# gvtulder/elasticdeform

Measured on AMD Instinct MI355X. Metric: Mvoxels/s fwd+grad, 256^3 fp32 order=3, higher is better.
Workload: dtype f32; 1 GPU; cfg2: 3D 256x256x256 float32, 5x5x5 grid sigma 5, order 3, mode mirror, prefilter on, deform_grid + deform_grid_gradient per step, one volume per GPU; parallelism=1 volume per GPU, no collective

## Files before the change

### elasticdeform_amd/csrc/deform_hot.hip

```cpp
#include <hip/hip_runtime.h>

#include <type_traits>

#include "ed_device.h"
#include "ed_params.h"
#include "ed_tile.h"

#ifndef ED_K2_U1
#define ED_K2_U1 1
#endif
#ifndef ED_K2_U2
#define ED_K2_U2 1
#endif
#define ED_PRAGMA(x) _Pragma(#x)
#define ED_UNROLL(n) ED_PRAGMA(unroll n)

namespace ed {
namespace tile {

namespace {

constexpr int kGradBoxBytes = 24 * 1024;

__device__ __forceinline__ void box_reduce_to_lds(int* red, int lane, int (&lo)[3], int (&hi)[3])
{
    box_reduce<6>(lo, hi);
    if (lane == 63) {
        const unsigned addr = (unsigned)(size_t)(__attribute__((address_space(3))) void*)red;
        asm volatile("ds_min_i32 %0, %1\n\t"
                     "ds_min_i32 %0, %2 offset:4\n\t"
                     "ds_min_i32 %0, %3 offset:8\n\t"
                     "ds_max_i32 %0, %4 offset:12\n\t"
                     "ds_max_i32 %0, %5 offset:16\n\t"
                     "ds_max_i32 %0, %6 offset:20"
                     :
                     : "v"(addr), "v"(lo[0]), "v"(lo[1]), "v"(lo[2]), "v"(hi[0]), "v"(hi[1]), "v"(hi[2])
                     : "memory");
    }
}
__device__ __forceinline__ float load_dy(const float* dy, long long off, int io16)
{
    return io16 ? widen16(reinterpret_cast<const unsigned short*>(dy)[off], io16) : dy[off];
}

__device__ __forceinline__ void hot_prologue(const HotGeom& hg, const Strip& sp, char* smem, int tid,
                                             bool copy_q = true, int nthreads = kBlock)
{
    int* sred = reinterpret_cast<int*>(smem + kOffRed);
    {
        const int* src = reinterpret_cast<const int*>(hg.xt + sp.tx0 * kT);
        int* dst = reinterpret_cast<int*>(smem + kOffTabX);
        const int avail = (hg.out_len[2] - sp.tx0 * kT) * 12;
        for (int e = tid; e < kStrip * kT * 12; e += nthreads)
            dst[e] = e < avail ? src[e] : 0;
    }
    if (copy_q && tid < 256) {
        const int row16 = 2 * hg.ncpx;
        const int r = tid >> 2;
        const int oz = min(sp.tz * kT + (r >> 3), hg.out_len[0] - 1);
        const int oy = min(sp.ty * kT + (r & 7), hg.out_len[1] - 1);
        const long long qrow_id = hg.q_strips > 1
                                      ? ((long long)oz * hg.out_len[1] + oy) * hg.q_strips + sp.tx0 / hg.strip_tiles
                                      : (long long)oz * hg.out_len[1] + oy;
        const double2* src = reinterpret_cast<const double2*>(
            hg.q + sp.sample * hg.q_bstride + qrow_id * (4 * hg.ncpx));
        double2* dst = reinterpret_cast<double2*>(smem + kOffQ) + r * row16;
        for (int k = tid & 3; k < row16; k += 4)
            dst[k] = src[k];
    }
    if (tid < 24) {
        const int k = tid & 7;
        sred[tid] = k < 3 ? 0x7fffffff : (int)0x80000000;
    }
    if (tid >= 128 && tid < 128 + 12)
        fill_hot_params(reinterpret_cast<HotParams*>(smem + kOffHot), hg, tid - 128);
    __syncthreads();
}

template <int ORDER, bool AFFINE>
__device__ __forceinline__ bool hot_coords(const HotGeom& hg, const HotParams* hp, const char* qrow,
                                           const double (&tw)[4], const int (&tib)[4], const int (&b)[3],
                                           const double (&P)[3], int* start, float* frac)
{
    double d[3];
    qrow_disp(qrow, tib, tw, d);
    return tile_coords<ORDER, AFFINE, float>(hg.in_len, &hg.mode, hp->period, hp->inv_period, d, b, P, start, frac);
}

template <int ORDER, bool AFFINE, int GRAD_WAVES, int TX, int NGRP = 1, bool IO16 = false>
__global__ __launch_bounds__(kBlock * NGRP, GRAD_WAVES) void hot_grad_kernel(const HotGeom hg)
{
    const int io16 = IO16 ? hg.io16 : 0;
    constexpr int NT = ORDER + 1;
    constexpr int NV = TX / 4, ZSTEP = 8 / NV;
    extern __shared__ __attribute__((aligned(16))) char smem0[];
    const int grp = NGRP == 2 ? (int)(threadIdx.x >> 8) : 0;
    const int tid = threadIdx.x & (kBlock - 1);
    char* smem = smem0 + grp * hg.lds_grp;
    int phase = 0;
    Strip sp;
    const int bidx = NGRP == 2 ? (int)(((blockIdx.x >> 3) * 2 + grp) * 8 + (blockIdx.x & 7)) : (int)blockIdx.x;
    if (!strip_of_block(hg, sp, bidx))
        return;
    for (int e = tid * 4; e < hg.box_cap; e += kBlock * 4)
        *reinterpret_cast<int4*>(smem + hg.off_box + e * 4) = make_int4(0, 0, 0, 0);
    hot_prologue(hg, sp, smem, tid);
    if (ED_DBG(hg.dbg, 8192))
        return;
    if (NGRP == 2 && grp == 1)
        __syncthreads();

    const AxTab* tabx = reinterpret_cast<const AxTab*>(smem + kOffTabX);
    int* sred = reinterpret_cast<int*>(smem + kOffRed);
    const HotParams* hp = reinterpret_cast<const HotParams*>(smem + kOffHot);
    int* box = reinterpret_cast<int*>(smem + hg.off_box);

    const int lane = tid & 63;
    const int wave = tid >> 6;
    const int zq = tid / (TX * 8);
    const bool rows16 = TX == 16 && ED_DBG(hg.dbg, 1 << 21);
    const int xx = (TX == 16 && !rows16) ? 2 * (tid & 7) + ((tid >> 4) & 1) : (tid & (TX - 1));
    const int yy = (TX == 16 && !rows16) ? 4 * ((tid >> 6) & 1) + ((tid >> 5) & 1) + 2 * ((tid >> 3) & 1) : ((tid / TX) & 7);
    const int ntile = (sp.ntile * kT + TX - 1) / TX;
    float* dx = hg.vol_w + sp.sample * hg.vol_bstride;
    const float* __restrict__ dy = hg.img_r + sp.sample * hg.img_bstride;

    const int oy = sp.ty * kT + yy;
    const char* qrow0 = smem + kOffQ + (zq * kT + yy) * (32 * hg.ncpx);
    const int qstep = ZSTEP * kT * 32 * hg.ncpx;
    const int oz0 = sp.tz * kT + zq;
    const bool vy = oy < hg.out_len[1];

    auto load_raw = [&](long long off) -> float {
        if constexpr (IO16)
            return __uint_as_float((unsigned)reinterpret_cast<const unsigned short*>(dy)[off]);
        else
            return dy[off];
    };
    float gnext[NV];
    {
        const int ox = sp.tx0 * kT + xx;
#pragma unroll
        for (int i = 0; i < NV; ++i)
            gnext[i] = (vy && ox < hg.out_len[2] && oz0 + ZSTEP * i < hg.out_len[0])
                           ? load_raw((oz0 + ZSTEP * i) * hg.img_sz + oy * hg.img_sy + ox) : 0.f;
    }
    int half = -1, half_next = -1;
    for (int ti = 0; ti < ntile; half = half_next, half_next = half == 0 ? 1 : -1, ti += half < 0 ? 1 : 0) {
        int* red = sred + (ti % 3) * 8;
        const int ox = sp.tx0 * kT + ti * TX + xx;
        const bool vx = ox < hg.out_len[2];
        const int ooff0 = oz0 * hg.img_sz + oy * hg.img_sy + ox;
        const int ostep = ZSTEP * hg.img_sz;

        float gpre[NV];
        if (half >= 0) {
#pragma unroll
            for (int i = 0; i < NV; ++i)
                gpre[i] = (vy && vx && oz0 + ZSTEP * i < hg.out_len[0]) ? load_raw(ooff0 + i * ostep) : 0.f;
        } else {
#pragma unroll
            for (int i = 0; i < NV; ++i)
                gpre[i] = gnext[i];
        }
        if (half < 0 && ti + 1 < ntile) {
            const bool nvx = ox + TX < hg.out_len[2];
#pragma unroll
            for (int i = 0; i < NV; ++i)
                gnext[i] = (vy && nvx && oz0 + ZSTEP * i < hg.out_len[0]) ? load_raw(ooff0 + TX + i * ostep) : 0.f;
        }
        const bool given = hg.use_boxes != 0;
        int gb0[3] = {0, 0, 0}, gbhi[3] = {-1, -1, -1};
        if (given) {
            const int t0 = sp.sample * hg.ntiles + (sp.tz * hg.tiles[1] + sp.ty) * hg.tiles[2] + sp.tx0 +
                           ti * (TX / kT);
            const int* bx = hg.boxes + (size_t)t0 * 8;
#pragma unroll
            for (int h = 0; h < 3; ++h) {
                gb0[h] = uni(bx[h]);
                gbhi[h] = uni(bx[3 + h]);
            }
            if (half < 0) {
#pragma unroll
                for (int k = 1; k < TX / kT; ++k) {
                    if (sp.tx0 + ti * (TX / kT) + k < hg.tiles[2]) {
#pragma unroll
                        for (int h = 0; h < 3; ++h) {
                            gb0[h] = min(gb0[h], uni(bx[k * 8 + h]));
                            gbhi[h] = max(gbhi[h], uni(bx[k * 8 + 3 + h]));
                        }
                    }
                }
            } else if (half == 1) {
#pragma unroll
                for (int h = 0; h < 3; ++h) {
                    gb0[h] = uni(bx[8 + h]);
                    gbhi[h] = uni(bx[8 + 3 + h]);
                }
            }
        }

        double tw[4];
        int tib[4];
        {
            const AxTab& t = tabx[ti * TX + xx];
#pragma unroll
            for (int l = 0; l < 4; ++l) {
                tw[l] = t.w[l];
                tib[l] = t.idx[l] * 8;
            }
        }
        double Pxy[3] = {0.0, 0.0, 0.0};
        if (AFFINE) {
#pragma unroll
            for (int h = 0; h < 3; ++h)
                Pxy[h] = fma(hp->affine[h * 4 + 2], (double)ox,
                             fma(hp->affine[h * 4 + 1], (double)oy, hp->affine[h * 4 + 3] + hp->offd[h]));
        }
        auto voxel = [&](int i, int* start, float* frac) -> bool {
            const int oz = oz0 + ZSTEP * i;
            const int b[3] = {oz + hg.off[0], oy + hg.off[1], ox + hg.off[2]};
            double P[3] = {0.0, 0.0, 0.0};
            if (AFFINE) {
#pragma unroll
                for (int h = 0; h < 3; ++h)
                    P[h] = fma(hp->affine[h * 4 + 0], (double)oz, Pxy[h]);
            }
            const bool cst = hot_coords<ORDER, AFFINE>(hg, hp, qrow0 + i * qstep, tw, tib, b, P, start, frac);
            return vy && vx && oz < hg.out_len[0] && !cst && (half < 0 || (xx >> 3) == half);
        };
        int lo[3] = {0x7fffffff, 0x7fffffff, 0x7fffffff};
        int hi[3] = {(int)0x80000000, (int)0x80000000, (int)0x80000000};
        if (!given) {
ED_UNROLL(ED_K2_U1)
            for (int i = 0; i < NV; ++i) {
                int start[3];
                float frac[3];
                if (voxel(i, start, frac)) {
#pragma unroll
                    for (int h = 0; h < 3; ++h) {
                        lo[h] = min(lo[h], start[h]);
                        hi[h] = max(hi[h], start[h] + ORDER);
                    }
                }
            }
        }
        float gval[NV];
        {
            float gm = 0.f;
#pragma unroll
            for (int i = 0; i < NV; ++i) {
                gval[i] = IO16 ? widen16(__float_as_uint(gpre[i]), io16) : gpre[i];
                gm += (__float_as_int(gval[i]) & 0x7f800000) == 0x7f800000 ? 0.f : fabsf(gval[i]);
            }
            gm = wave_sum(gm);
            if (lane == 0)
                reinterpret_cast<float*>(smem + kOffSum)[(phase & 1) * 4 + wave] = gm;
        }
        if (!given)
            box_reduce_to_lds(red, lane, lo, hi);
        lds_barrier();
        int b0[3], bhi[3];
        if (given) {
#pragma unroll
            for (int h = 0; h < 3; ++h) {
                b0[h] = gb0[h];
                bhi[h] = gbhi[h];
            }
        } else {
#pragma unroll
            for (int h = 0; h < 3; ++h) {
                b0[h] = uni(red[h]);
                bhi[h] = uni(red[3 + h]);
            }
        }
        bool any = bhi[0] >= b0[0] && bhi[1] >= b0[1] && bhi[2] >= b0[2];
        if (given && !any) {
            b0[0] = b0[1] = b0[2] = 0;
            bhi[0] = bhi[1] = bhi[2] = -1;
            any = true;
        }
        const int ext[3] = {bhi[0] - b0[0] + 1, bhi[1] - b0[1] + 1, bhi[2] - b0[2] + 1};
        if (tid < 6 && !given)
            sred[((ti + 2) % 3) * 8 + tid] = tid < 3 ? 0x7fffffff : (int)0x80000000;
        if (!any)
            continue;
        int pitch = ext[2] <= 8 ? 8 : (ext[2] <= 24 ? 24 : (ext[2] <= 40 ? 40 : (ext[2] <= 56 ? 56 : 0)));
        if (ED_DBG(hg.dbg, 1024))
            pitch = ext[2] <= 16 ? 16 : (ext[2] <= 48 ? 48 : 0);
        if (ED_DBG(hg.dbg, 1 << 22))
            pitch = ext[2] <= 32 ? 32 : 0;
        if (given && ((unsigned)ext[0] > 4096u || (unsigned)ext[1] > 4096u))
            pitch = 0;
        const int by = ext[1];
        const int nrows = ext[0] * by;
        const int nbox = nrows * pitch;
        if (hg.hint && tid == 0 && half < 0 && (pitch == 0 || nbox > hg.small_cap))
            atomicAdd(hg.hint, (hg.large_cap > 0 && (pitch == 0 || nbox > hg.large_cap)) ? kHintHuge * (TX / kT) : TX / kT);
        bool direct_tile = false;
        if (pitch == 0 || nbox > hg.box_cap) {
            if (TX == 16 && given && half < 0 && sp.tx0 + ti * 2 + 1 < hg.tiles[2]) {
                half_next = 0;
                continue;
            }
            if (hg.self_serve) {
                direct_tile = true;
            } else {
                const int t8 = sp.tx0 + ti * (TX / kT) + (half >= 0 ? half : tid);
                if (tid < (half >= 0 ? 1 : TX / kT) && t8 < hg.tiles[2]) {
                    const int slot = atomicAdd(&hg.spill[0], 1);
                    hg.spill[1 + slot] = sp.sample * hg.ntiles + (sp.tz * hg.tiles[1] + sp.ty) * hg.tiles[2] + t8;
                }
                continue;
            }
        }
        const bool interior = b0[0] >= 0 && b0[0] + ext[0] <= hg.in_len[0] && b0[1] >= 0 &&
                              b0[1] + ext[1] <= hg.in_len[1] && b0[2] >= 0 && b0[2] + ext[2] <= hg.in_len[2];

        for (long long ss = 0; ss < hg.nsteps; ++ss, ++phase) {
            long long vol_off = 0, img_off = 0;
            if (hg.nstep)
                hot_step_offsets(hp, ss, vol_off, img_off);
            float* dst = dx + vol_off;
            float* gsum = reinterpret_cast<float*>(smem + kOffSum) + (phase & 1) * 4;
            if (ss > 0) {
                float gm = 0.f;
#pragma unroll
                for (int i = 0; i < NV; ++i) {
                    const bool inb = vy && vx && oz0 + ZSTEP * i < hg.out_len[0];
                    gval[i] = inb ? load_dy(dy, img_off + ooff0 + i * ostep, io16) : 0.f;
                    gm += (__float_as_int(gval[i]) & 0x7f800000) == 0x7f800000 ? 0.f : fabsf(gval[i]);
                }
                gm = wave_sum(gm);
                if (lane == 0)
                    gsum[wave] = gm;
                lds_barrier();
            }
            const float gtot = unif((gsum[0] + gsum[1]) + (gsum[2] + gsum[3]));
            constexpr float kC = (float)((2147483648.0 - 1024.0) /
                                         ((ORDER == 1 ? 1.0 : ORDER == 2 ? 0.4219 : ORDER == 3 ? 0.2963
                                           : ORDER == 4 ? 0.2150 : 0.1664) * 1.001));
            const float scale = gtot > 0.f ? fminf(kC * __frcp_rn(gtot), 3.0e38f) : 0.f;
            const float inv_scale = gtot > 0.f ? __frcp_rn(scale) : 0.f;

ED_UNROLL(ED_K2_U2)
            for (int i = 0; i < NV; ++i) {
                float gv = gval[0];
#pragma unroll
                for (int k = 1; k < NV; ++k)
                    gv = i == k ? gval[k] : gv;
                if (gv == 0.f || ED_DBG(hg.dbg, 128))
                    continue;
                int st[3];
                float fr[3];
                if (!voxel(i, st, fr))
                    continue;
                float w0[NT], w1[NT], w2[NT];
                weights_from_frac<float, ORDER>(fr[0], w0);
                weights_from_frac<float, ORDER>(fr[1], w1);
                weights_from_frac<float, ORDER>(fr[2], w2);
                const int rz = st[0] - b0[0], ry = st[1] - b0[1], rx = st[2] - b0[2];
                const bool outside = direct_tile || (given && (rz < 0 || rz + ORDER >= ext[0] || ry < 0 || ry + ORDER >= ext[1] ||
                                                               rx < 0 || rx + ORDER >= ext[2]));
                if ((__float_as_int(gv) & 0x7f800000) == 0x7f800000 || outside) {
#pragma unroll 1
                    for (int t = 0; t < NT * NT * NT; ++t) {
                        const int l0 = t / (NT * NT), l1 = (t / NT) % NT, l2 = t % NT;
                        const int zs = mirror_i32(st[0] + l0, hg.in_len[0]);
                        const int ys = mirror_i32(st[1] + l1, hg.in_len[1]);
                        const int xs = mirror_i32(st[2] + l2, hg.in_len[2]);
                        float wp = w0[0], wq = w1[0], wr = w2[0];
#pragma unroll
                        for (int l = 1; l < NT; ++l) {
                            wp = l0 == l ? w0[l] : wp;
                            wq = l1 == l ? w1[l] : wq;
                            wr = l2 == l ? w2[l] : wr;
                        }
                        unsafeAtomicAdd(dst + (zs * hg.vol_sz + ys * hg.vol_sy + xs), gv * wp * wq * wr);
                    }
                    continue;
                }
                int* bp = box + (rz * by + ry) * pitch + rx;
                const float gs = gv * scale;
#pragma unroll
                for (int l0 = 0; l0 < NT; ++l0) {
                    const float g0 = gs * w0[l0];
#pragma unroll
                    for (int l1 = 0; l1 < NT; ++l1) {
                        const float g1 = g0 * w1[l1];
                        int* rp = bp + (l0 * by + l1) * pitch;
                        typedef float f2_t __attribute__((ext_vector_type(2)));
                        float pr[NT + 1];
#pragma unroll
                        for (int l2 = 0; l2 + 1 < NT + 1; l2 += 2) {
                            const f2_t wv = {w2[l2], l2 + 1 < NT ? w2[l2 + 1] : 0.f};
                            const f2_t gg = {g1, g1};
                            const f2_t pv = wv * gg;
                            pr[l2] = pv.x;
                            pr[l2 + 1] = pv.y;
                        }
#pragma unroll
                        for (int l2 = 0; l2 < NT; ++l2)
                            atomicAdd(reinterpret_cast<unsigned*>(rp + l2), (unsigned)round_half_up_i32(pr[l2]));
                    }
                }
            }
            lds_barrier();
            {
                constexpr int FL = TX == 8 ? 16 : 32;
                constexpr int FR = kBlock / FL;
                constexpr int FU = 4;
                const int sub = tid & (FL - 1);
                const int rslot = tid / FL;
                const float inv_by = 1.f / (float)by;
                const int nr = (ED_DBG(hg.dbg, 64) || direct_tile) ? 0 : nrows;
                const int dz8 = (int)(((float)FR + 0.5f) * inv_by), dy8 = FR - dz8 * by;
                const int step8 = dz8 * hg.vol_sz + dy8 * hg.vol_sy, wrapfix = hg.vol_sz - by * hg.vol_sy;
                for (int xo = 0; xo < ext[2]; xo += FL) {
                    const int xi = xo + sub;
                    const bool xin = xi < ext[2];
                    const int xs = interior ? xi : mirror_i32(b0[2] + xi, hg.in_len[2]);
                    int zr = (int)(((float)rslot + 0.5f) * inv_by), yr = rslot - zr * by;
                    int rowoff = (b0[0] + zr) * hg.vol_sz + (b0[1] + yr) * hg.vol_sy + b0[2];
                    for (int r0 = rslot; r0 < nr; r0 += FU * FR) {
                        int acc[FU];
#pragma unroll
                        for (int k = 0; k < FU; ++k) {
                            const int r = r0 + k * FR;
                            acc[k] = (xin && r < nr) ? __hip_atomic_exchange(&box[r * pitch + xi], 0, __ATOMIC_RELAXED,
                                                                             __HIP_MEMORY_SCOPE_WORKGROUP)
                                                     : 0;
                        }
#pragma unroll
                        for (int k = 0; k < FU; ++k) {
                            if (ED_DBG(hg.dbg, 4096) ? acc[k] == 0x7ffffff1 : acc[k] != 0) {
                                int off = rowoff;
                                if (!interior)
                                    off = mirror_i32(b0[0] + zr, hg.in_len[0]) * hg.vol_sz +
                                          mirror_i32(b0[1] + yr, hg.in_len[1]) * hg.vol_sy;
                                unsafeAtomicAdd(dst + (off + xs), (float)acc[k] * inv_scale);
                            }
                            yr += dy8;
                            zr += dz8;
                            rowoff += step8;
                            if (yr >= by) {
                                yr -= by;
                                zr += 1;
                                rowoff += wrapfix;
                            }
                        }
                    }
                }
            }
        }
    }
}

template <int ORDER>
hipError_t launch_grad_order(const HotGeom& hg, unsigned nblk, size_t lds, hipStream_t stream)
{
#ifdef EDHIP_EXPERIMENTS
    const int duo = ed_env("EDHIP_GRAD_DUO") ? atoi(ed_env("EDHIP_GRAD_DUO")) : 0;
    if (duo && !hg.has_affine && ORDER == 3) {
        if constexpr (ORDER == 3) {
            auto kern = hot_grad_kernel<ORDER, false, 4, 16, 2>;
            static bool once = false;
            if (!once) {
                (void)hipFuncSetAttribute(reinterpret_cast<const void*>(kern),
                                          hipFuncAttributeMaxDynamicSharedMemorySize, 160 * 1024);
                once = true;
            }
            const unsigned per = nblk / 8;
            hipLaunchKernelGGL(kern, dim3(8 * ((per + 1) / 2)), dim3(2 * kBlock), 2 * (size_t)hg.lds_grp, stream, hg);
        }
        return hipGetLastError();
    }
#endif
    auto go = [&](auto kern, unsigned& raised_on) -> hipError_t {
        if (lds > 64 * 1024) {
            int dev = 0;
            (void)hipGetDevice(&dev);
            const unsigned bit = 1u << (dev & 31);
            if (!(__atomic_load_n(&raised_on, __ATOMIC_RELAXED) & bit)) {
                const hipError_t e = hipFuncSetAttribute(reinterpret_cast<const void*>(kern),
                                                         hipFuncAttributeMaxDynamicSharedMemorySize, 160 * 1024);
                if (e != hipSuccess)
                    return e;
                __atomic_fetch_or(&raised_on, bit, __ATOMIC_RELAXED);
            }
        }
        hipLaunchKernelGGL(kern, dim3(nblk), dim3(kBlock), lds, stream, hg);
        return hipGetLastError();
    };
    static unsigned raised[4] = {0, 0, 0, 0};
    if (hg.io16) {
        if constexpr (ORDER <= 3) {
            if (hg.has_affine)
                return go(hot_grad_kernel<ORDER, true, 4, 16, 1, true>, raised[0]);
            return go(hot_grad_kernel<ORDER, false, 4, 16, 1, true>, raised[1]);
        }
        return hipErrorNotSupported;
    }
    if (hg.has_affine)
        return go(hot_grad_kernel<ORDER, true, 4, 16>, raised[2]);
    return go(hot_grad_kernel<ORDER, false, 4, 16>, raised[3]);
}

}

size_t hot_lds_bytes(bool gradient, int ncpx, int* box_cap, int* off_box, int level)
{
    const size_t q = (size_t)kT * kT * 32 * (size_t)ncpx;
    const size_t off = (kOffQ + q + 15) & ~(size_t)15;
    *off_box = (int)off;
    const bool large = level >= 1;
    if (gradient) {
        size_t box = level >= 2 ? 64 * 1024 : (large ? 36 * 1024 : kGradBoxBytes);
        if (const char* kb = ed_env("EDHIP_GRAD_BOX_KB"))
            box = (size_t)atoi(kb) * 1024;
        *box_cap = (int)(box / 4);
        const size_t total = off + box;
        return total <= 80 * 1024 ? total : 0;
    }
    size_t budget = large ? 52 * 1024 : 40 * 1024;
    if (off + 2 * 4 * 2488 > budget)
        budget = 64 * 1024;
    if (off + 2 * 4 * 2488 > budget)
        return 0;
    size_t cap = (budget - off) / 8;
    cap = ((cap - 56) / 64) * 64 + 56;
    *box_cap = (int)cap;
    return off + 2 * 4 * cap;
}

hipError_t launch_hot_grad_level1(const HotGeom& hg, int order, unsigned nblk, size_t lds, hipStream_t stream)
{
    switch (order) {
    case 1: return launch_grad_order<1>(hg, nblk, lds, stream);
    case 2: return launch_grad_order<2>(hg, nblk, lds, stream);
    case 3: return launch_grad_order<3>(hg, nblk, lds, stream);
    case 4: return launch_grad_order<4>(hg, nblk, lds, stream);
    case 5: return launch_grad_order<5>(hg, nblk, lds, stream);
    default: return hipErrorNotSupported;
    }
}

}
}
```

Measured before the change: 26340 Mvoxels/s.

## Add software-pipelined coordinate/weight compute interleaved with LDS scatter in grad kernel

Result: no change. 26400 Mvoxels/s, median of 5 (+0.2%).

```diff
diff --git a/elasticdeform_amd/csrc/deform_hot.hip b/elasticdeform_amd/csrc/deform_hot.hip
--- a/elasticdeform_amd/csrc/deform_hot.hip
+++ b/elasticdeform_amd/csrc/deform_hot.hip
@@ -1,6 +1,7 @@
 #include <hip/hip_runtime.h>
 
 #include <type_traits>
+#include <utility>
 
 #include "ed_device.h"
 #include "ed_params.h"
@@ -11,6 +12,9 @@
 #endif
 #ifndef ED_K2_U2
 #define ED_K2_U2 1
+#endif
+#ifndef ED_K2_PIPE
+#define ED_K2_PIPE 0
 #endif
 #define ED_PRAGMA(x) _Pragma(#x)
 #define ED_UNROLL(n) ED_PRAGMA(unroll n)
@@ -37,6 +41,16 @@
                      : "v"(addr), "v"(lo[0]), "v"(lo[1]), "v"(lo[2]), "v"(hi[0]), "v"(hi[1]), "v"(hi[2])
                      : "memory");
     }
+}
+template <int... I, class F>
+__device__ __forceinline__ void static_for_seq(std::integer_sequence<int, I...>, F&& f)
+{
+    (f(std::integral_constant<int, I>{}), ...);
+}
+template <int N, class F>
+__device__ __forceinline__ void static_for(F&& f)
+{
+    static_for_seq(std::make_integer_sequence<int, N>{}, f);
 }
 __device__ __forceinline__ float load_dy(const float* dy, long long off, int io16)
 {
@@ -84,7 +98,27 @@
 {
     double d[3];
     qrow_disp(qrow, tib, tw, d);
-    return tile_coords<ORDER, AFFINE, float>(hg.in_len, &hg.mode, hp->period, hp->inv_period, d, b, P, start, frac);
+    int ci[3];
+    bool inr[3];
+#pragma unroll
+    for (int h = 0; h < 3; ++h)
+        inr[h] = coord_axis_fast<ORDER, float>(AFFINE ? P[h] + d[h] : d[h], AFFINE ? 0 : b[h], hg.in_len[h], ci[h], frac[h]);
+    bool cst = false;
+    if (!(inr[0] && inr[1] && inr[2])) {
+#pragma unroll
+        for (int h = 0; h < 3; ++h) {
+            if (!inr[h]) {
+                int len = hg.in_len[h];
+                asm volatile("" : "+s"(len));
+                cst = coord_axis_mapped<ORDER, float>(AFFINE ? P[h] + d[h] : (double)b[h] + d[h], len, hg.mode, hp->period[h],
+                                                      hp->inv_period[h], ci[h], frac[h]) || cst;
+            }
+        }
+    }
+#pragma unroll
+    for (int h = 0; h < 3; ++h)
+        start[h] = cst ? 0 : ci[h] - ORDER / 2;
+    return cst;
 }
 
 template <int ORDER, bool AFFINE, int GRAD_WAVES, int TX, int NGRP = 1, bool IO16 = false>
@@ -93,6 +127,7 @@
     const int io16 = IO16 ? hg.io16 : 0;
     constexpr int NT = ORDER + 1;
     constexpr int NV = TX / 4, ZSTEP = 8 / NV;
+    constexpr bool kPipe = ED_K2_PIPE && !AFFINE && !IO16 && ORDER <= 3 && NGRP == 1;
     extern __shared__ __attribute__((aligned(16))) char smem0[];
     const int grp = NGRP == 2 ? (int)(threadIdx.x >> 8) : 0;
     const int tid = threadIdx.x & (kBlock - 1);
@@ -316,6 +351,9 @@
         }
         const bool interior = b0[0] >= 0 && b0[0] + ext[0] <= hg.in_len[0] && b0[1] >= 0 &&
                               b0[1] + ext[1] <= hg.in_len[1] && b0[2] >= 0 && b0[2] + ext[2] <= hg.in_len[2];
+        const bool full_tile = kPipe && interior && !direct_tile && half < 0 && sp.tz * kT + kT <= hg.out_len[0] &&
+                               sp.ty * kT + kT <= hg.out_len[1] && sp.tx0 * kT + (ti + 1) * TX <= hg.out_len[2] &&
+                               ext[0] > ORDER && ext[1] > ORDER && ext[2] > ORDER;
 
         for (long long ss = 0; ss < hg.nsteps; ++ss, ++phase) {
             long long vol_off = 0, img_off = 0;
@@ -343,13 +381,156 @@
             const float scale = gtot > 0.f ? fminf(kC * __frcp_rn(gtot), 3.0e38f) : 0.f;
             const float inv_scale = gtot > 0.f ? __frcp_rn(scale) : 0.f;
 
+            auto scatter_direct = [&](float gv, const int (&st)[3], const float (&w0)[NT], const float (&w1)[NT],
+                                      const float (&w2)[NT]) {
+#pragma unroll 1
+                for (int t = 0; t < NT * NT * NT; ++t) {
+                    const int l0 = t / (NT * NT), l1 = (t / NT) % NT, l2 = t % NT;
+                    const int zs = mirror_i32(st[0] + l0, hg.in_len[0]);
+                    const int ys = mirror_i32(st[1] + l1, hg.in_len[1]);
+                    const int xs = mirror_i32(st[2] + l2, hg.in_len[2]);
+                    float wp = w0[0], wq = w1[0], wr = w2[0];
+#pragma unroll
+                    for (int l = 1; l < NT; ++l) {
+                        wp = l0 == l ? w0[l] : wp;
+                        wq = l1 == l ? w1[l] : wq;
+                        wr = l2 == l ? w2[l] : wr;
+                    }
+                    unsafeAtomicAdd(dst + (zs * hg.vol_sz + ys * hg.vol_sy + xs), gv * wp * wq * wr);
+                }
+            };
+            auto scatter_row = [&](int* bp, float gs, int l0, int l1, const float (&w0)[NT], const float (&w1)[NT],
+                                   const float (&w2)[NT]) {
+                const float g0 = gs * w0[l0];
+                const float g1 = g0 * w1[l1];
+                int* rp = bp + (l0 * by + l1) * pitch;
+                typedef float f2_t __attribute__((ext_vector_type(2)));
+                float pr[NT + 1];
+#pragma unroll
+                for (int l2 = 0; l2 + 1 < NT + 1; l2 += 2) {
+                    const f2_t wv = {w2[l2], l2 + 1 < NT ? w2[l2 + 1] : 0.f};
+                    const f2_t gg = {g1, g1};
+                    const f2_t pv = wv * gg;
+                    pr[l2] = pv.x;
+                    pr[l2 + 1] = pv.y;
+                }
+#pragma unroll
+                for (int l2 = 0; l2 < NT; ++l2)
+                    atomicAdd(reinterpret_cast<unsigned*>(rp + l2), (unsigned)round_half_up_i32(pr[l2]));
+            };
+            unsigned todo = (1u << NV) - 1u;
+            if (kPipe && full_tile) {
+                struct Stage {
+                    double2 q01;
+                    double q2;
+                    double d[3];
+                    float fr[3];
+                    int r[3];
+                    float w0[NT], w1[NT], w2[NT];
+                    int cell;
+                    float gs;
+                    bool defer;
+                };
+                constexpr int kSlices = 10, kRows = NT * NT;
+                const int lim[3] = {ext[0] - 1 - ORDER, ext[1] - 1 - ORDER, ext[2] - 1 - ORDER};
+                auto slice = [&](auto sl_c, int i, float gv, Stage& n) {
+                    constexpr int sl = decltype(sl_c)::value;
+                    const char* qrow = qrow0 + i * qstep;
+                    auto read = [&](int l) {
+                        n.q01 = *reinterpret_cast<const double2*>(qrow + tib[l]);
+                        n.q2 = *reinterpret_cast<const double*>(qrow + tib[l] + 16);
+                    };
+                    if constexpr (sl == 0) {
+                        read(0);
+                    } else if constexpr (sl == 1) {
+                        n.d[0] = tw[0] * n.q01.x;
+                        n.d[1] = tw[0] * n.q01.y;
+                        n.d[2] = tw[0] * n.q2;
+                        read(1);
+                    } else if constexpr (sl <= 4) {
+                        n.d[0] = fma(tw[sl - 1], n.q01.x, n.d[0]);
+                        n.d[1] = fma(tw[sl - 1], n.q01.y, n.d[1]);
+                        n.d[2] = fma(tw[sl - 1], n.q2, n.d[2]);
+                        if constexpr (sl < 4)
+                            read(sl);
+                    } else if constexpr (sl == 5) {
+                        const int b[3] = {oz0 + ZSTEP * i + hg.off[0], oy + hg.off[1], ox + hg.off[2]};
+#pragma unroll
+                        for (int h = 0; h < 3; ++h) {
+                            int ci;
+                            (void)coord_axis_fast<ORDER, float>(n.d[h], b[h], hg.in_len[h], ci, n.fr[h]);
+                            n.r[h] = ci - ORDER / 2 - b0[h];
+                        }
+                    } else if constexpr (sl == 6) {
+                        const bool ok = (n.r[0] >= 0) & (n.r[0] <= lim[0]) & (n.r[1] >= 0) & (n.r[1] <= lim[1]) &
+                                        (n.r[2] >= 0) & (n.r[2] <= lim[2]) &
+                                        ((__float_as_int(gv) & 0x7f800000) != 0x7f800000);
+                        const int keep = -(int)ok;
+                        n.cell = (__mul24(__mul24(n.r[0], by) + n.r[1], pitch) + n.r[2]) & keep;
+                        n.gs = __int_as_float(__float_as_int(gv * scale) & keep);
+                        n.defer = !ok;
+                    } else if constexpr (sl == 7) {
+                        weights_from_frac<float, ORDER>(n.fr[0], n.w0);
+                    } else if constexpr (sl == 8) {
+                        weights_from_frac<float, ORDER>(n.fr[1], n.w1);
+                    } else {
+                        weights_from_frac<float, ORDER>(n.fr[2], n.w2);
+                    }
+                };
+                Stage cur;
+                static_for<kSlices>([&](auto sl) { slice(sl, 0, gval[0], cur); });
+                unsigned deferred = cur.defer ? 1u : 0u;
+#if ED_K2_PIPE == 1
+                static_for<NV>([&](auto ic) {
+                    constexpr int i = decltype(ic)::value;
+                    if constexpr (i > 0) {
+                        static_for<kSlices>([&](auto sl) { slice(sl, i, gval[i], cur); });
+                        deferred |= cur.defer ? 1u << i : 0u;
+                    }
+                    static_for<kRows>([&](auto gc) {
+                        constexpr int g = decltype(gc)::value;
+                        scatter_row(box + cur.cell, cur.gs, g / NT, g % NT, cur.w0, cur.w1, cur.w2);
+                    });
+                });
+#else
+                static_for<NV>([&](auto ic) {
+                    constexpr int i = decltype(ic)::value;
+                    Stage nxt;
+                    static_for<kRows>([&](auto gc) {
+                        constexpr int g = decltype(gc)::value;
+                        __builtin_amdgcn_sched_barrier(0);
+                        if constexpr (i + 1 < NV) {
+                            static_for<kSlices>([&](auto sl) {
+                                if constexpr (decltype(sl)::value * kRows / kSlices == g)
+                                    slice(sl, i + 1, gval[i + 1 < NV ? i + 1 : 0], nxt);
+                            });
+                        }
+                        asm volatile("" : "+v"(cur.cell), "+v"(cur.gs));
+                        scatter_row(box + cur.cell, cur.gs, g / NT, g % NT, cur.w0, cur.w1, cur.w2);
+                    });
+                    if constexpr (i + 1 < NV) {
+                        deferred |= nxt.defer ? 2u << i : 0u;
+#pragma unroll
+                        for (int l = 0; l < NT; ++l) {
+                            cur.w0[l] = nxt.w0[l];
+                            cur.w1[l] = nxt.w1[l];
+                            cur.w2[l] = nxt.w2[l];
+                        }
+                        cur.cell = nxt.cell;
+                        cur.gs = nxt.gs;
+                    }
+                });
+#endif
+                __builtin_amdgcn_sched_barrier(0);
+                todo = deferred;
+            }
 ED_UNROLL(ED_K2_U2)
             for (int i = 0; i < NV; ++i) {
                 float gv = gval[0];
 #pragma unroll
                 for (int k = 1; k < NV; ++k)
                     gv = i == k ? gval[k] : gv;
-                if (gv == 0.f || ED_DBG(hg.dbg, 128))
+                if (!((todo >> i) & 1u) || gv == 0.f || ED_DBG(hg.dbg, 128))
                     continue;
                 int st[3];
                 float fr[3];
@@ -363,46 +544,16 @@
                 const bool outside = direct_tile || (given && (rz < 0 || rz + ORDER >= ext[0] || ry < 0 || ry + ORDER >= ext[1] ||
                                                                rx < 0 || rx + ORDER >= ext[2]));
                 if ((__float_as_int(gv) & 0x7f800000) == 0x7f800000 || outside) {
-#pragma unroll 1
-                    for (int t = 0; t < NT * NT * NT; ++t) {
-                        const int l0 = t / (NT * NT), l1 = (t / NT) % NT, l2 = t % NT;
-                        const int zs = mirror_i32(st[0] + l0, hg.in_len[0]);
-                        const int ys = mirror_i32(st[1] + l1, hg.in_len[1]);
-                        const int xs = mirror_i32(st[2] + l2, hg.in_len[2]);
-                        float wp = w0[0], wq = w1[0], wr = w2[0];
-#pragma unroll
-                        for (int l = 1; l < NT; ++l) {
-                            wp = l0 == l ? w0[l] : wp;
-                            wq = l1 == l ? w1[l] : wq;
-                            wr = l2 == l ? w2[l] : wr;
-                        }
-                        unsafeAtomicAdd(dst + (zs * hg.vol_sz + ys * hg.vol_sy + xs), gv * wp * wq * wr);
-                    }
+                    scatter_direct(gv, st, w0, w1, w2);
                     continue;
                 }
                 int* bp = box + (rz * by + ry) * pitch + rx;
                 const float gs = gv * scale;
 #pragma unroll
                 for (int l0 = 0; l0 < NT; ++l0) {
-                    const float g0 = gs * w0[l0];
-#pragma unroll
-                    for (int l1 = 0; l1 < NT; ++l1) {
-                        const float g1 = g0 * w1[l1];
-                        int* rp = bp + (l0 * by + l1) * pitch;
-                        typedef float f2_t __attribute__((ext_vector_type(2)));
-                        float pr[NT + 1];
-#pragma unroll
-                        for (int l2 = 0; l2 + 1 < NT + 1; l2 += 2) {
-                            const f2_t wv = {w2[l2], l2 + 1 < NT ? w2[l2 + 1] : 0.f};
-                            const f2_t gg = {g1, g1};
-                            const f2_t pv = wv * gg;
-                            pr[l2] = pv.x;
-                            pr[l2 + 1] = pv.y;
-                        }
-#pragma unroll
-                        for (int l2 = 0; l2 < NT; ++l2)
-                            atomicAdd(reinterpret_cast<unsigned*>(rp + l2), (unsigned)round_half_up_i32(pr[l2]));
-                    }
+#pragma unroll
+                    for (int l1 = 0; l1 < NT; ++l1)
+                        scatter_row(bp, gs, l0, l1, w0, w1, w2);
                 }
             }
             lds_barrier();
@@ -410,8 +561,10 @@
                 constexpr int FL = TX == 8 ? 16 : 32;
                 constexpr int FR = kBlock / FL;
                 constexpr int FU = 4;
-                const int sub = tid & (FL - 1);
-                const int rslot = tid / FL;
+                int ftid = tid;
+                asm volatile("" : "+v"(ftid));
+                const int sub = ftid & (FL - 1);
+                const int rslot = ftid / FL;
                 const float inv_by = 1.f / (float)by;
                 const int nr = (ED_DBG(hg.dbg, 64) || direct_tile) ? 0 : nrows;
                 const int dz8 = (int)(((float)FR + 0.5f) * inv_by), dy8 = FR - dz8 * by;
```
